# ingra14m/RobIR

Hardware: AMD Instinct MI355X
Metric: PBR-stage rays/sec (128 SG lobes, 32 visibility samples/lobe), full forward render (higher is better)
Workload: dtype f32 (every MLP -- light visibility, SDF values and reverse-mode gradient, colour, visibility, 512-wide and CESR nets: every fp32 operand exact as three f16 pieces, six MFMA products per multiply-add in three fp32 accumulators -- in the light-visibility kernel the two outer products of the 2^-22 clas

## Files before the change

robir_amd/csrc/vis_diffuse_x6t.hip:

```cpp
#include "../../include/robir_hip.h"
#include "common.h"
#include "mlp_engine.h"
#include "x6_ring.h"

namespace rb {

#define RB_TINY 1e-6f
constexpr int XT_MAX_DIRS = 4096;
constexpr int XT_WF4 = 1536;
constexpr int XT_CF4 = 4 + XT_WF4;
constexpr int XT_SLOTS = 4, XT_DIST = 3;
constexpr int XT_PIECES = 6;
#ifndef XT_FP8
#define XT_FP8 1
#endif

__device__ __forceinline__ void xt_dma16(const f4* gbase_uniform, unsigned lane_byte_off, unsigned lds_byte_uniform) {
  asm volatile("s_mov_b32 m0, %0\n\ts_nop 0\n\tglobal_load_lds_dwordx4 %1, %2" ::"s"(lds_byte_uniform), "v"(lane_byte_off),
               "s"(gbase_uniform)
               : "memory");
}
template <int OFF>
__device__ __forceinline__ void xt_dma16_imm(const f4* gbase_uniform, unsigned lane_byte_off, unsigned lds_byte_uniform) {
  asm volatile("s_mov_b32 m0, %0\n\ts_nop 0\n\tglobal_load_lds_dwordx4 %1, %2 offset:%3" ::"s"(lds_byte_uniform), "v"(lane_byte_off),
               "s"(gbase_uniform), "n"(OFF)
               : "memory");
}

template <int OFF>
__device__ __forceinline__ void xt_dma16_m0kept(const f4* gbase_uniform, unsigned lane_byte_off) {
  asm volatile("global_load_lds_dwordx4 %0, %1 offset:%2" ::"v"(lane_byte_off), "s"(gbase_uniform), "n"(OFF) : "memory");
}

struct XtTile {
  int point;
  int dir_base;
};
struct XtArgs {
  const float *A, *Bd;
  const f4* W49;
  int argmax_vis;
  unsigned* range_word;
  const float *normals, *dirs, *wdir, *wsum;
  const int* cid;
  int L, nsamp;
  float* vis_out;
  unsigned long long* eval_count;
  const unsigned short* pair_j;
  const XtTile* tile_info;
  const unsigned long long* counters;
  float* pair_vis;
};

template <bool STREAM>
__global__ __launch_bounds__(256, 1) void k_dvis_x6t(const XtArgs a) {
  __shared__ f4 ring[XT_SLOTS * XT_WF4];
  __shared__ f4 headw[XT_WF4];
  __shared__ f4 bias_tab[49 * 4];
  __shared__ f4 aux[(XT_MAX_DIRS * 4 + XT_MAX_DIRS * 2) / 16 + 64];
  __shared__ int s_count;
  float* const vis_tab = reinterpret_cast<float*>(aux);
  unsigned short* const idx_list = reinterpret_cast<unsigned short*>(aux + XT_MAX_DIRS / 4);
  f4* const a_row = aux + (XT_MAX_DIRS * 6) / 16;
  f4* const a_rows = aux;
  const float* __restrict__ A = a.A;
  const float* __restrict__ Bd = a.Bd;
  const f4* __restrict__ W49 = a.W49;
  const int argmax_vis = a.argmax_vis;
  const int tid = threadIdx.x, lane = tid & 63, g = lane >> 4;
  const int wave = __builtin_amdgcn_readfirstlane(tid >> 6);
  const float negk = -2048.0f;
  constexpr float C11 = 1.0f / 2048.0f;
  const long p = blockIdx.x;
  const int L = a.L, nsamp = a.nsamp, LS = L * nsamp;
  long dbase = 0;
  int S = 0, rounds = 0;
  const int G = gridDim.x;
  long total_tiles = 0, total_rounds = 0;
  for (int i = tid; i < 49 * 4; i += 256) bias_tab[i] = W49[(long)(i >> 2) * XT_CF4 + (i & 3)];
  for (int i = tid; i < XT_WF4; i += 256) headw[i] = W49[48L * XT_CF4 + 4 + i];
  if constexpr (STREAM) {
    total_tiles = (long)a.counters[0];
    total_rounds = (total_tiles + 7) >> 3;
    __syncthreads();
    if ((long)blockIdx.x >= total_rounds) return;
    rounds = 1;
  } else {
  const float* __restrict__ normals = a.normals;
  const float* __restrict__ dirs = a.dirs;
  const int* __restrict__ cid = a.cid;
  dbase = (cid ? (long)cid[p] : 0L) * LS;
  if (tid == 0) s_count = 0;
  if (tid < 64) a_row[tid] = reinterpret_cast<const f4*>(A + p * 256)[tid];
  for (int j = tid; j < LS; j += 256) vis_tab[j] = 0.f;
  __syncthreads();
  const float nx = normals[3 * p], ny = normals[3 * p + 1], nz = normals[3 * p + 2];
  for (int j0 = 0; j0 < LS; j0 += 256) {
    const int j = j0 + tid;
    bool front = false;
    if (j < LS) {
      const float* d = dirs + 3 * (dbase + j);
      const float c = nx * d[0] + ny * d[1] + nz * d[2];
      front = c > RB_TINY;
    }
    const unsigned long long mk = __ballot(front);
    int base = 0;
    if (lane == 0 && mk) base = atomicAdd(&s_count, __popcll(mk));
    base = __shfl(base, 0);
    if (front) idx_list[base + __popcll(mk & ((1ull << lane) - 1ull))] = (unsigned short)j;
  }
  __syncthreads();
  S = s_count;
  if (tid == 0 && a.eval_count) atomicAdd(a.eval_count, (unsigned long long)S);
  rounds = (S + 127) / 128;
  }

  const unsigned ring_b = (unsigned)(unsigned long)((__attribute__((address_space(3))) char*)ring);
  unsigned voff_a = (unsigned)wave * 6144u + (unsigned)lane * 16u, voff_b = voff_a + 4096u;
  asm volatile("" : "+v"(voff_a), "+v"(voff_b));
  const unsigned wave_lds = ring_b + (unsigned)wave * 6144u;
  typedef const __attribute__((address_space(3))) u4* lds_u4p;
  unsigned ring_a0 = ring_b + (unsigned)lane * 16u, ring_a2 = ring_a0 + 2u * XT_WF4 * 16u;
  asm volatile("" : "+v"(ring_a0), "+v"(ring_a2));
  const lds_u4p ring_u = (lds_u4p)ring_a0, ring_u2 = (lds_u4p)ring_a2;
  u4 wh[4], wm[4], wl[4];
#if XT_FP8
  typedef int xt_i8 __attribute__((ext_vector_type(8)));
  xt_i8 w8h, w8l;
#define XT_F16OFF(KB, PIECE) (((KB) >> 2) * 768 + (((KB) & 3) * 2 + (PIECE)) * 64)
#define XT_LOAD8(DST, BASE, OFF)                                                                                             \
  {                                                                                                                          \
    const u4 a_ = (BASE)[(OFF)], b_ = (BASE)[(OFF) + 64];                                                                    \
    DST = xt_i8{(int)a_[0], (int)a_[1], (int)a_[2], (int)a_[3], (int)b_[0], (int)b_[1], (int)b_[2], (int)b_[3]};             \
  }
#endif
  f4 bias;
  if (rounds > 0) {
#pragma unroll
    for (int c = 0; c < 3; ++c)
#pragma unroll
      for (int i = 0; i < XT_PIECES; ++i)
        xt_dma16(W49 + (long)c * XT_CF4 + 4 + i * 64, voff_a, wave_lds + (unsigned)c * 24576u + (unsigned)i * 1024u);
    asm volatile("s_waitcnt vmcnt(12)" ::: "memory");
    __builtin_amdgcn_s_barrier();
    asm volatile("" ::: "memory");
#pragma unroll
    for (int k = 0; k < 4; ++k) {
#if XT_FP8
      wh[k] = ring_u[XT_F16OFF(k, 0)];
      wm[k] = ring_u[XT_F16OFF(k, 1)];
#else
      wh[k] = ring_u[(k * 3 + 0) * 64];
      wm[k] = ring_u[(k * 3 + 1) * 64];
      wl[k] = ring_u[(k * 3 + 2) * 64];
#endif
    }
#if XT_FP8
    XT_LOAD8(w8h, ring_u, 512)
    XT_LOAD8(w8l, ring_u, 640)
#endif
    bias = bias_tab[g];
  }

  unsigned sat = 0u;
#if XT_FP8
  struct Ops {
    u4 h[2][8], m[2][8];
    xt_i8 h8[2][2], l8[2][2];
  };
  unsigned el_keep[2] = {0u, 0u};
#else
  struct Ops {
    u4 h[2][8], m[2][8], l[2][8];
  };
#endif
  Ops P, Q;

#define XT_MFMA(ACC, WREG, XREG) \
  ACC = __builtin_amdgcn_mfma_f32_16x16x32_f16(__builtin_bit_cast(h8, WREG), __builtin_bit_cast(h8, XREG), ACC, 0, 0, 0)

  float ev0[2][2], ev1[2][2], ed0, ed1;
  unsigned eh;
  SxAcc prev[2];
  auto ep_stage1 = [&](int t, int q) {
    const SxAcc& a = prev[t];
    const float r0 = __builtin_fmaf(__builtin_fmaf(a.c2[2 * q], C11, a.c1[2 * q]), C11, a.c0[2 * q]);
    const float r1 = __builtin_fmaf(__builtin_fmaf(a.c2[2 * q + 1], C11, a.c1[2 * q + 1]), C11, a.c0[2 * q + 1]);
    ev0[t][q] = fmaxf(r0, 0.f);
    ev1[t][q] = fmaxf(r1, 0.f);
  };
  auto ep_stage2 = [&](int t, int q) {
    const unsigned hu = __builtin_bit_cast(unsigned, __builtin_amdgcn_cvt_pkrtz(ev0[t][q], ev1[t][q]));
    const float s0 = ev0[t][q] * 2048.0f, s1 = ev1[t][q] * 2048.0f;
    asm("v_fma_mix_f32 %0, %1, %2, %3 op_sel_hi:[1,0,0]" : "=v"(ed0) : "v"(hu), "s"(negk), "v"(s0));
    asm("v_fma_mix_f32 %0, %1, %2, %3 op_sel:[1,0,0] op_sel_hi:[1,0,0]" : "=v"(ed1) : "v"(hu), "s"(negk), "v"(s1));
    eh = hu;
    sat = sat_acc_nonneg(sat, hu);
  };
  auto ep_stage3 = [&](Ops& Y, int t, int jb, int q) {
    const unsigned mu = __builtin_bit_cast(unsigned, __builtin_amdgcn_cvt_pkrtz(ed0, ed1));
    const float e0 = ed0 * 2048.0f, e1 = ed1 * 2048.0f;
    unsigned lu;
    asm("v_fma_mixlo_f16 %0, %1, %2, %3 op_sel_hi:[1,0,0]" : "=v"(lu) : "v"(mu), "s"(negk), "v"(e0));
    asm("v_fma_mixhi_f16 %0, %1, %2, %3 op_sel:[1,0,0] op_sel_hi:[1,0,0]" : "+v"(lu) : "v"(mu), "s"(negk), "v"(e1));
    Y.h[t][jb >> 1][(jb & 1) * 2 + q] = eh;
    Y.m[t][jb >> 1][(jb & 1) * 2 + q] = mu;
#if XT_FP8
    if (q == 0) {
      el_keep[t] = lu;
    } else {
      Y.h8[t][jb >> 3][jb & 7] = (int)__builtin_amdgcn_perm(eh, Y.h[t][jb >> 1][(jb & 1) * 2], 0x07050301u);
      Y.l8[t][jb >> 3][jb & 7] = (int)__builtin_amdgcn_perm(lu, el_keep[t], 0x07050301u);
    }
#else
    Y.l[t][jb >> 1][(jb & 1) * 2 + q] = lu;
#endif
  };
  auto ep_slot = [&](Ops& Y, int s, int pj) {
    switch (s) {
      case 0: ep_stage1(0, 0); break;
      case 1: ep_stage1(0, 1); break;
      case 2: ep_stage1(1, 0); break;
      case 3: ep_stage1(1, 1); break;
      case 4: ep_stage2(0, 0); break;
      case 5: ep_stage3(Y, 0, pj, 0); break;
      case 6: ep_stage2(0, 1); break;
      case 7: ep_stage3(Y, 0, pj, 1); break;
      case 8: ep_stage2(1, 0); break;
      case 9: ep_stage3(Y, 1, pj, 0); break;
      case 10: ep_stage2(1, 1); break;
      default: ep_stage3(Y, 1, pj, 1); break;
    }
  };

  f4 raw[2][16];
  int jj[2], jjn[2];
  int tpn[2] = {-1, -1}, tbn[2] = {0, 0}, jn2[2] = {0xFFFF, 0xFFFF};
  const unsigned arow_b = (unsigned)(unsigned long)((__attribute__((address_space(3))) char*)a_rows);
  XtTile recn[2] = {{-1, 0}, {-1, 0}};
  bool okn[2] = {false, false};
  auto tile_lookup = [&](long round) {
#pragma unroll
    for (int t = 0; t < 2; ++t) {
      const long T = round * 8 + wave * 2 + t;
      okn[t] = round < total_rounds && T < total_tiles;
      const long Tc = T < total_tiles ? T : total_tiles - 1;
      recn[t] = a.tile_info[Tc];
      jn2[t] = (int)a.pair_j[Tc * 16 + (lane & 15)];
    }
  };
  auto tile_resolve = [&]() {
#pragma unroll
    for (int t = 0; t < 2; ++t) {
      tpn[t] = okn[t] ? __builtin_amdgcn_readfirstlane(recn[t].point) : -1;
      tbn[t] = okn[t] ? __builtin_amdgcn_readfirstlane(recn[t].dir_base) : 0;
      if (!okn[t]) jn2[t] = 0xFFFF;
    }
  };
  auto fetch_rows = [&](long rd_next, int parity_next) {
    if constexpr (STREAM) {
      tile_resolve();
#pragma unroll
      for (int t = 0; t < 2; ++t) {
        const long prow = tpn[t] < 0 ? 0L : (long)tpn[t];
        xt_dma16(reinterpret_cast<const f4*>(A + prow * 256), (unsigned)lane * 16u,
                 arow_b + (unsigned)(parity_next * 8 + wave * 2 + t) * 1024u);
      }
    }
#pragma unroll
    for (int t = 0; t < 2; ++t) {
      long row;
      if constexpr (STREAM) {
        jjn[t] = (tpn[t] < 0 || jn2[t] == 0xFFFF) ? -1 : jn2[t];
        row = (long)tbn[t] + (jjn[t] < 0 ? 0 : jjn[t]);
      } else {
        const int si = (int)rd_next * 128 + t * 64 + wave * 16 + (lane & 15);
        jjn[t] = si < S ? (int)idx_list[si] : -1;
        row = dbase + (jjn[t] < 0 ? 0 : jjn[t]);
      }
      const f4* brow = reinterpret_cast<const f4*>(Bd + row * 256) + g;
#pragma unroll
      for (int kb = 0; kb < 16; ++kb) raw[t][kb] = brow[kb * 4];
    }
  };
  long rd = STREAM ? (long)blockIdx.x : 0L;
  const long rd_end = STREAM ? total_rounds : (long)rounds, rd_step = STREAM ? (long)G : 1L;
  int parity = 0;
  if constexpr (STREAM) tile_lookup(rd);
  if (rounds > 0) fetch_rows(rd, 0);
#ifdef XT_TIMING
#define XT_T(i) { const unsigned long long t_ = __builtin_amdgcn_s_memtime(); tacc[i] += t_ - tlast; tlast = t_; }
  unsigned long long tacc[4] = {0, 0, 0, 0}, tlast = __builtin_amdgcn_s_memtime();
  int trounds = 0;
#else
#define XT_T(i)
#endif
  for (; rd < rd_end; rd += rd_step) {
    if constexpr (STREAM) tile_lookup(rd + rd_step);
#ifdef XT_TIMING
    ++trounds;
#endif
    XT_T(3)
#pragma unroll
    for (int t = 0; t < 2; ++t) {
      jj[t] = jjn[t];
      const f4* arow = STREAM ? a_rows + (parity * 8 + wave * 2 + t) * 64 : a_row;
#pragma unroll
      for (int kb = 0; kb < 16; ++kb) {
        const f4 bv = raw[t][kb];
        const f4 av = arow[kb * 4 + g];
#pragma unroll
        for (int q = 0; q < 2; ++q) {
          unsigned h, m, l;
          sx_split_pair(fmaxf(av[2 * q] + bv[2 * q], 0.f), fmaxf(av[2 * q + 1] + bv[2 * q + 1], 0.f), negk, h, m, l);
          P.h[t][kb / 2][(kb & 1) * 2 + q] = h;
          P.m[t][kb / 2][(kb & 1) * 2 + q] = m;
#if XT_FP8
          if (q == 0) {
            el_keep[t] = l;
          } else {
            P.h8[t][kb >> 3][kb & 7] = (int)__builtin_amdgcn_perm(h, P.h[t][kb / 2][(kb & 1) * 2], 0x07050301u);
            P.l8[t][kb >> 3][kb & 7] = (int)__builtin_amdgcn_perm(l, el_keep[t], 0x07050301u);
          }
#else
          P.l[t][kb / 2][(kb & 1) * 2 + q] = l;
#endif
          sat = sat_acc_nonneg(sat, h);
        }
      }
    }
    XT_T(0)
    auto layer = [&](int l, Ops& X, Ops& Y) {
      const f4* Wl = W49 + (long)l * 16 * XT_CF4 + 4;
      const f4* Wn = W49 + (long)(l == 2 ? 0 : l + 1) * 16 * XT_CF4 + 4;
#pragma unroll
      for (int jb = 0; jb < 16; ++jb) {
        SxAcc acc[2];
        asm volatile("s_waitcnt vmcnt(6)" ::: "memory");
#ifndef XT_ABL_NOBAR
        __builtin_amdgcn_s_barrier();
#endif
        asm volatile("" ::: "memory");
        const int nx3 = jb + XT_DIST;
        const f4* dsrc = nx3 < 16 ? Wl + (long)nx3 * XT_CF4 : Wn + (long)(nx3 - 16) * XT_CF4;
        const unsigned ddst = wave_lds + (unsigned)(nx3 & 3) * 24576u;
        const f4 nbias = bias_tab[(l * 16 + jb + 1) * 4 + g];
#if defined(XT_ABL_NODMA)
#define XT_COPY(I) do { } while (0)
#else
#define XT_COPY(I)                                                                  \
  do {                                                                              \
    if ((I) == 0) xt_dma16_imm<0>(dsrc, voff_a, ddst);                              \
    else if ((I) < 4) xt_dma16_m0kept<((I) & 3) * 1024>(dsrc, voff_a);              \
    else if ((I) == 4) xt_dma16_imm<0>(dsrc, voff_b, ddst + 4096u);                 \
    else xt_dma16_m0kept<((I) & 3) * 1024>(dsrc, voff_b);                           \
  } while (0)
#endif
#define XT_FENCE __builtin_amdgcn_sched_barrier(0)
#ifdef XT_ABL_NOLDS
#define XT_FRAG(DST, KB, PIECE) asm volatile("" : "+v"(DST))
#else
#if XT_FP8
#define XT_FRAG(DST, KB, PIECE) DST = nfrag[XT_F16OFF(KB, PIECE)]
#else
#define XT_FRAG(DST, KB, PIECE) DST = nfrag[((KB) * 3 + (PIECE)) * 64]
#endif
#endif
#define XT_MFMA8(ACC, WREG, XREG) ACC = __builtin_amdgcn_mfma_scale_f32_16x16x128_f8f6f4(WREG, XREG, ACC, 1, 1, 0, 0, 0, 0)
#define XT_EP(S)                        \
  do {                                  \
    if (jb > 0) ep_slot(Y, (S), jb - 1); \
  } while (0)
#define XT_RUN(ACC, WP, XP)                     \
  _Pragma("unroll") for (int k_ = 0; k_ < 4; ++k_) { \
    const int k = H ? 3 - k_ : k_;               \
    XT_MFMA(ACC, WP[k], XP[4 * H + k]);          \
  }
#define XT_RUN_REFILL(ACC, WP, XP, PIECE)          \
  _Pragma("unroll") for (int k_ = 0; k_ < 4; ++k_) { \
    const int k = H ? 3 - k_ : k_;                   \
    XT_MFMA(ACC, WP[k], XP[4 * H + k]);              \
    XT_FRAG(WP[k], 4 * (1 - H) + k, PIECE);          \
  }
#pragma unroll
        for (int H = 0; H < 2; ++H) {
          const lds_u4p nfrag = (((jb + H) & 2) ? ring_u2 : ring_u) + ((jb + H) & 1) * XT_WF4;
          if (H == 0) {
            acc[0].c0 = bias;
            acc[1].c0 = bias;
            acc[0].c1 = acc[0].c2 = acc[1].c1 = acc[1].c2 = f4{0.f, 0.f, 0.f, 0.f};
          }
          XT_RUN(acc[0].c0, wh, X.h[0]);
          if (H == 0) XT_EP(0); else XT_EP(9);
          XT_FENCE;
          XT_RUN(acc[0].c1, wh, X.m[0]);
          if (H == 0) XT_EP(1); else XT_EP(10);
          XT_FENCE;
#if XT_FP8
          XT_MFMA8(acc[0].c2, w8h, X.l8[0][H]);
          if (H == 0) XT_EP(2); else XT_EP(11);
          XT_FENCE;
          XT_RUN(acc[1].c0, wh, X.h[1]);
          if (H == 0) XT_EP(3); else XT_COPY(0);
          XT_FENCE;
          XT_RUN_REFILL(acc[1].c1, wh, X.m[1], 0);
          XT_FENCE;
          XT_MFMA8(acc[1].c2, w8h, X.l8[1][H]);
#ifndef XT_ABL_NOLDS
          XT_LOAD8(w8h, nfrag, (1 - H) * 768 + 512)
#endif
          if (H == 0) XT_EP(4); else XT_COPY(1);
          XT_FENCE;
#else
          XT_RUN(acc[0].c2, wh, X.l[0]);
          if (H == 0) XT_EP(2); else XT_EP(11);
          XT_FENCE;
          XT_RUN(acc[1].c0, wh, X.h[1]);
          if (H == 0) XT_EP(3); else XT_COPY(0);
          XT_FENCE;
          XT_RUN(acc[1].c1, wh, X.m[1]);
          if (H == 0) XT_EP(4); else XT_COPY(1);
          XT_FENCE;
          XT_RUN_REFILL(acc[1].c2, wh, X.l[1], 0);
          XT_FENCE;
#endif
          XT_RUN(acc[0].c1, wm, X.h[0]);
          if (H == 0) XT_EP(5); else XT_COPY(2);
          XT_FENCE;
          XT_RUN(acc[0].c2, wm, X.m[0]);
          if (H == 0) XT_EP(6); else XT_COPY(3);
          XT_FENCE;
          XT_RUN(acc[1].c1, wm, X.h[1]);
          if (H == 0) XT_EP(7); else XT_COPY(4);
          XT_FENCE;
          XT_RUN_REFILL(acc[1].c2, wm, X.m[1], 1);
          XT_FENCE;
#if XT_FP8
          XT_MFMA8(acc[0].c2, w8l, X.h8[0][H]);
          if (H == 0) XT_EP(8); else XT_COPY(5);
          XT_FENCE;
          XT_MFMA8(acc[1].c2, w8l, X.h8[1][H]);
#ifndef XT_ABL_NOLDS
          XT_LOAD8(w8l, nfrag, (1 - H) * 768 + 640)
#endif
          XT_FENCE;
#else
          XT_RUN(acc[0].c2, wl, X.h[0]);
          if (H == 0) XT_EP(8); else XT_COPY(5);
          XT_FENCE;
          XT_RUN_REFILL(acc[1].c2, wl, X.h[1], 2);
          XT_FENCE;
#endif
        }
#undef XT_RUN
#undef XT_RUN_REFILL
#undef XT_COPY
#undef XT_FENCE
#undef XT_FRAG
#undef XT_MFMA8
#undef XT_EP
        prev[0] = acc[0];
        prev[1] = acc[1];
        bias = nbias;
      }
#pragma unroll
      for (int s = 0; s < 12; ++s) ep_slot(Y, s, 15);
    };
#pragma unroll 1
    for (int l = 0; l < 3; ++l) {
      layer(l, P, Q);
#pragma unroll
      for (int t = 0; t < 2; ++t)
#pragma unroll
        for (int kb = 0; kb < 8; ++kb) {
          P.h[t][kb] = Q.h[t][kb];
          P.m[t][kb] = Q.m[t][kb];
#if !XT_FP8
          P.l[t][kb] = Q.l[t][kb];
#endif
        }
#if XT_FP8
#pragma unroll
      for (int t = 0; t < 2; ++t)
#pragma unroll
        for (int hf = 0; hf < 2; ++hf) {
          P.h8[t][hf] = Q.h8[t][hf];
          P.l8[t][hf] = Q.l8[t][hf];
        }
#endif
    }
    XT_T(1)
    if constexpr (STREAM) fetch_rows(rd + rd_step, parity ^ 1);
    else fetch_rows(rd + 1 < rd_end ? rd + 1 : rd, 0);
    {
      const u4* hw = reinterpret_cast<const u4*>(headw) + lane;
      SxAcc acc[2];
#pragma unroll
      for (int t = 0; t < 2; ++t) {
        acc[t].c0 = bias;
        acc[t].c1 = f4{0.f, 0.f, 0.f, 0.f};
        acc[t].c2 = f4{0.f, 0.f, 0.f, 0.f};
      }
#pragma unroll
#if XT_FP8
      for (int kb = 0; kb < 8; ++kb) {
        const u4 fh = hw[XT_F16OFF(kb, 0)], fm = hw[XT_F16OFF(kb, 1)];
#pragma unroll
        for (int t = 0; t < 2; ++t) {
          XT_MFMA(acc[t].c0, fh, P.h[t][kb]);
          XT_MFMA(acc[t].c1, fh, P.m[t][kb]);
          XT_MFMA(acc[t].c1, fm, P.h[t][kb]);
          XT_MFMA(acc[t].c2, fm, P.m[t][kb]);
        }
      }
#pragma unroll
      for (int hf = 0; hf < 2; ++hf) {
        xt_i8 f8h, f8l;
        XT_LOAD8(f8h, hw, hf * 768 + 512)
        XT_LOAD8(f8l, hw, hf * 768 + 640)
#pragma unroll
        for (int t = 0; t < 2; ++t) {
          acc[t].c2 = __builtin_amdgcn_mfma_scale_f32_16x16x128_f8f6f4(f8h, P.l8[t][hf], acc[t].c2, 1, 1, 0, 0, 0, 0);
          acc[t].c2 = __builtin_amdgcn_mfma_scale_f32_16x16x128_f8f6f4(f8l, P.h8[t][hf], acc[t].c2, 1, 1, 0, 0, 0, 0);
        }
      }
#else
      for (int kb = 0; kb < 8; ++kb) {
        const u4 fh = hw[(kb * 3 + 0) * 64], fm = hw[(kb * 3 + 1) * 64], fl = hw[(kb * 3 + 2) * 64];
#pragma unroll
        for (int t = 0; t < 2; ++t) {
          XT_MFMA(acc[t].c0, fh, P.h[t][kb]);
          XT_MFMA(acc[t].c1, fh, P.m[t][kb]);
          XT_MFMA(acc[t].c2, fh, P.l[t][kb]);
          XT_MFMA(acc[t].c1, fm, P.h[t][kb]);
          XT_MFMA(acc[t].c2, fm, P.m[t][kb]);
          XT_MFMA(acc[t].c2, fl, P.h[t][kb]);
        }
      }
#endif
      bias = bias_tab[g];
#pragma unroll
      for (int t = 0; t < 2; ++t) {
        const float l0 = __builtin_fmaf(__builtin_fmaf(acc[t].c2[0], C11, acc[t].c1[0]), C11, acc[t].c0[0]);
        const float l1 = __builtin_fmaf(__builtin_fmaf(acc[t].c2[1], C11, acc[t].c1[1]), C11, acc[t].c0[1]);
        if (g == 0 && jj[t] >= 0) {
          float v;
          if (argmax_vis) {
            v = l1 > l0 ? 1.f : 0.f;
          } else {
            const float mx = fmaxf(l0, l1);
            const float e0 = expf(l0 - mx), e1 = expf(l1 - mx);
            v = e1 / (e0 + e1);
          }
          if constexpr (STREAM) a.pair_vis[(rd * 8 + wave * 2 + t) * 16 + (lane & 15)] = v;
          else vis_tab[jj[t]] = v;
        }
      }
    }
    parity ^= 1;
    XT_T(2)
  }
#ifdef XT_TIMING
  if ((blockIdx.x == 7 || blockIdx.x == 4000) && tid == 0 && trounds > 0)
    printf("x6t wg %d rounds %d cycles/round: conv %llu layers %llu head+fetch %llu lookup %llu\n", (int)blockIdx.x, trounds, tacc[0] / trounds,
           tacc[1] / trounds, tacc[2] / trounds, tacc[3] / trounds);
#endif
#undef XT_MFMA
  range_report<true>(sat, a.range_word);
  asm volatile("s_waitcnt vmcnt(0)" ::: "memory");
  __syncthreads();
  if constexpr (!STREAM) {
    if (tid < L) {
      const float* w = a.wdir + dbase + (long)tid * nsamp;
      float acc = 0.f;
      for (int k = 0; k < nsamp; ++k) acc += vis_tab[tid * nsamp + k] * w[k];
      a.vis_out[p * L + tid] = acc / a.wsum[(a.cid ? a.cid[p] : 0) * L + tid];
    }
  }
}

struct V3Tile;
__global__ void k_dvis3_cull(const float* __restrict__ normals, const int* __restrict__ cid, long n, const float* __restrict__ dirs, int LS,
                             unsigned short* __restrict__ pair_j, V3Tile* __restrict__ tile_info, int2* __restrict__ point_info,
                             unsigned long long* __restrict__ counters, unsigned long long* __restrict__ eval_count);
__global__ void k_dvis3_reduce(const int* __restrict__ cid, long n, const float* __restrict__ wdir, const float* __restrict__ wsum,
                               const unsigned short* __restrict__ pair_j, const float* __restrict__ pair_vis,
                               const int2* __restrict__ point_info, int L, int nsamp, float* __restrict__ vis_out);

}

using namespace rb;

extern "C" int rb_dvis_fused_x6t(const float* normals, const int* chunk_id, long n, const float* A, const float* Bd,
                                 const float* dirs, const float* wdir, const float* wsum, const float* W49, int L, int nsamp,
                                 int argmax_vis, int scale_log2, float* vis_out, unsigned long long* eval_count,
                                 rb_stream_t stream) {
  if (n <= 0) return 0;
  RB_REQUIRE(normals && A && Bd && dirs && wdir && wsum && W49 && vis_out, "null pointer");
  RB_REQUIRE(n <= RB_MAX_BLOCKS, "too many points for one launch (one workgroup each)");
  RB_REQUIRE(L > 0 && L <= 256 && nsamp > 0 && (long)L * nsamp <= XT_MAX_DIRS, "need L <= 256 and L*nsamp <= 4096");
#if XT_FP8
  RB_REQUIRE(scale_log2 == 8, "this build of k_dvis_x6t takes the bf8 weight layout (packing.repack_x6_chunks_fp8; scale_log2 = 8 names it)");
#else
  RB_REQUIRE(scale_log2 == 0, "k_dvis_x6t takes weights packed with scale_log2 = 0");
#endif
  XtArgs a{};
  a.A = A, a.Bd = Bd, a.W49 = (const f4*)W49, a.argmax_vis = argmax_vis;
  a.range_word = range_flags() ? range_flags() + RB_RANGE_DVIS : nullptr;
  a.normals = normals, a.dirs = dirs, a.wdir = wdir, a.wsum = wsum, a.cid = chunk_id, a.L = L, a.nsamp = nsamp;
  a.vis_out = vis_out, a.eval_count = eval_count;
  hipLaunchKernelGGL(k_dvis_x6t<false>, dim3((unsigned)n), dim3(256), 0, (hipStream_t)stream, a);
  return check_launch("k_dvis_x6t");
}

extern "C" int rb_dvis_stream_x6(const float* normals, const int* chunk_id, long n, const float* A, const float* Bd,
                                 const float* dirs, const float* wdir, const float* wsum, const float* W49, int L, int nsamp,
                                 int argmax_vis, int scale_log2, unsigned short* pair_j, float* pair_vis, int* tile_info,
                                 int* point_info, unsigned long long* counters, int n_workgroups, float* vis_out,
                                 unsigned long long* eval_count, rb_stream_t stream) {
  if (n <= 0) return 0;
  RB_REQUIRE(normals && A && Bd && dirs && wdir && wsum && W49 && vis_out, "null pointer");
  RB_REQUIRE(pair_j && pair_vis && tile_info && point_info && counters, "null scratch pointer");
  RB_REQUIRE(n <= RB_MAX_BLOCKS, "too many points for one launch (one workgroup each in the cull / reduce passes)");
  RB_REQUIRE(L > 0 && L <= 256 && nsamp > 0 && (long)L * nsamp <= XT_MAX_DIRS && (L * nsamp) % 16 == 0,
             "need L <= 256, L*nsamp <= 4096 and a multiple of 16");
  RB_REQUIRE((long)n * (L * nsamp / 16) < (1L << 31), "tile index would overflow 31 bits");
#if XT_FP8
  RB_REQUIRE(scale_log2 == 8, "this build of k_dvis_x6t takes the bf8 weight layout (packing.repack_x6_chunks_fp8; scale_log2 = 8 names it)");
#else
  RB_REQUIRE(scale_log2 == 0, "k_dvis_x6t takes weights packed with scale_log2 = 0");
#endif
  hipStream_t s = (hipStream_t)stream;
  if (n_workgroups <= 0) n_workgroups = device_cus();
  RB_REQUIRE(n_workgroups > 0, "device query failed");
  if (hipMemsetAsync(counters, 0, 2 * sizeof(unsigned long long), s) != hipSuccess) return rb::fail(__func__, "memset failed");
  hipLaunchKernelGGL(k_dvis3_cull, dim3((unsigned)n), dim3(256), 0, s, normals, chunk_id, n, dirs, L * nsamp, pair_j,
                     reinterpret_cast<V3Tile*>(tile_info), reinterpret_cast<int2*>(point_info), counters, eval_count);
  if (int rc = check_launch("k_dvis3_cull")) return rc;
  XtArgs a{};
  a.A = A, a.Bd = Bd, a.W49 = (const f4*)W49, a.argmax_vis = argmax_vis;
  a.range_word = range_flags() ? range_flags() + RB_RANGE_DVIS : nullptr;
  a.pair_j = pair_j, a.tile_info = reinterpret_cast<const XtTile*>(tile_info), a.counters = counters, a.pair_vis = pair_vis;
  hipLaunchKernelGGL(k_dvis_x6t<true>, dim3((unsigned)n_workgroups), dim3(256), 0, s, a);
  if (int rc = check_launch("k_dvis_x6t<stream>")) return rc;
  hipLaunchKernelGGL(k_dvis3_reduce, dim3((unsigned)n), dim3(256), 0, s, chunk_id, n, wdir, wsum, pair_j, pair_vis,
                     reinterpret_cast<const int2*>(point_info), L, nsamp, vis_out);
  return check_launch("k_dvis3_reduce");
}
```

Baseline: 510,000.

## Overlap weight DMA with culling prologue and parallelize the visibility reduction

In the non-stream path, the per-point prologue is restructured. Direction, head-weight, bias and A-row loads are issued together into registers, and the weight-ring DMA starts before culling so global latency overlaps. The LDS atomic compaction is replaced by per-wave ballot counts and a prefix over waves, which produces a deterministic ordered index list with fewer barriers. The epilogue multiplies by wdir across all 256 threads before a short per-lobe sum, replacing serial strided global reads. This adds register pressure from the prefetched arrays and only applies when LS is at most 4096.

```diff
diff --git a/robir_amd/csrc/vis_diffuse_x6t.hip b/robir_amd/csrc/vis_diffuse_x6t.hip
--- a/robir_amd/csrc/vis_diffuse_x6t.hip
+++ b/robir_amd/csrc/vis_diffuse_x6t.hip
@@ -7,6 +7,7 @@
 
 #define RB_TINY 1e-6f
 constexpr int XT_MAX_DIRS = 4096;
+constexpr int XT_CULL_IT = XT_MAX_DIRS / 256;
 constexpr int XT_WF4 = 1536;
 constexpr int XT_CF4 = 4 + XT_WF4;
 constexpr int XT_SLOTS = 4, XT_DIST = 3;
@@ -58,7 +59,7 @@
   __shared__ f4 headw[XT_WF4];
   __shared__ f4 bias_tab[49 * 4];
   __shared__ f4 aux[(XT_MAX_DIRS * 4 + XT_MAX_DIRS * 2) / 16 + 64];
-  __shared__ int s_count;
+  __shared__ int s_count[4];
   float* const vis_tab = reinterpret_cast<float*>(aux);
   unsigned short* const idx_list = reinterpret_cast<unsigned short*>(aux + XT_MAX_DIRS / 4);
   f4* const a_row = aux + (XT_MAX_DIRS * 6) / 16;
@@ -77,42 +78,76 @@
   int S = 0, rounds = 0;
   const int G = gridDim.x;
   long total_tiles = 0, total_rounds = 0;
-  for (int i = tid; i < 49 * 4; i += 256) bias_tab[i] = W49[(long)(i >> 2) * XT_CF4 + (i & 3)];
-  for (int i = tid; i < XT_WF4; i += 256) headw[i] = W49[48L * XT_CF4 + 4 + i];
+#ifdef XT_TIMING
+  const unsigned long long tstart = __builtin_amdgcn_s_memtime();
+#endif
+  auto ring_start = [&](unsigned voff, unsigned wlds) {
+#pragma unroll
+    for (int c = 0; c < 3; ++c)
+#pragma unroll
+      for (int i = 0; i < XT_PIECES; ++i)
+        xt_dma16(W49 + (long)c * XT_CF4 + 4 + i * 64, voff, wlds + (unsigned)c * 24576u + (unsigned)i * 1024u);
+  };
   if constexpr (STREAM) {
+    for (int i = tid; i < 49 * 4; i += 256) bias_tab[i] = W49[(long)(i >> 2) * XT_CF4 + (i & 3)];
+    for (int i = tid; i < XT_WF4; i += 256) headw[i] = W49[48L * XT_CF4 + 4 + i];
     total_tiles = (long)a.counters[0];
     total_rounds = (total_tiles + 7) >> 3;
     __syncthreads();
     if ((long)blockIdx.x >= total_rounds) return;
     rounds = 1;
   } else {
-  const float* __restrict__ normals = a.normals;
-  const float* __restrict__ dirs = a.dirs;
-  const int* __restrict__ cid = a.cid;
-  dbase = (cid ? (long)cid[p] : 0L) * LS;
-  if (tid == 0) s_count = 0;
-  if (tid < 64) a_row[tid] = reinterpret_cast<const f4*>(A + p * 256)[tid];
-  for (int j = tid; j < LS; j += 256) vis_tab[j] = 0.f;
-  __syncthreads();
-  const float nx = normals[3 * p], ny = normals[3 * p + 1], nz = normals[3 * p + 2];
-  for (int j0 = 0; j0 < LS; j0 += 256) {
-    const int j = j0 + tid;
-    bool front = false;
-    if (j < LS) {
-      const float* d = dirs + 3 * (dbase + j);
-      const float c = nx * d[0] + ny * d[1] + nz * d[2];
-      front = c > RB_TINY;
-    }
-    const unsigned long long mk = __ballot(front);
+    const float* __restrict__ normals = a.normals;
+    const float* __restrict__ dirs = a.dirs;
+    const int* __restrict__ cid = a.cid;
+    dbase = (cid ? (long)cid[p] : 0L) * LS;
+    ring_start((unsigned)wave * 6144u + (unsigned)lane * 16u,
+               (unsigned)(unsigned long)((__attribute__((address_space(3))) char*)ring) + (unsigned)wave * 6144u);
+    const float nx = normals[3 * p], ny = normals[3 * p + 1], nz = normals[3 * p + 2];
+    float dx[XT_CULL_IT], dy[XT_CULL_IT], dz[XT_CULL_IT];
+#pragma unroll
+    for (int it = 0; it < XT_CULL_IT; ++it) {
+      const int j = it * 256 + tid;
+      const float* d = dirs + 3 * (dbase + (j < LS ? j : LS - 1));
+      dx[it] = d[0], dy[it] = d[1], dz[it] = d[2];
+    }
+    f4 hw_r[XT_WF4 / 256];
+#pragma unroll
+    for (int k = 0; k < XT_WF4 / 256; ++k) hw_r[k] = W49[48L * XT_CF4 + 4 + k * 256 + tid];
+    const int bi = tid < 49 * 4 ? tid : 49 * 4 - 1;
+    const f4 bias_r = W49[(long)(bi >> 2) * XT_CF4 + (bi & 3)];
+    const f4 arow_r = reinterpret_cast<const f4*>(A + p * 256)[lane];
+    for (int j = tid; j < LS; j += 256) vis_tab[j] = 0.f;
+    unsigned long long mk[XT_CULL_IT];
+    int wave_count = 0;
+#pragma unroll
+    for (int it = 0; it < XT_CULL_IT; ++it) {
+      const float c = nx * dx[it] + ny * dy[it] + nz * dz[it];
+      mk[it] = __ballot(it * 256 + tid < LS && c > RB_TINY);
+      wave_count += __popcll(mk[it]);
+    }
+    if (lane == 0) s_count[wave] = wave_count;
+#pragma unroll
+    for (int k = 0; k < XT_WF4 / 256; ++k) headw[k * 256 + tid] = hw_r[k];
+    if (tid < 49 * 4) bias_tab[tid] = bias_r;
+    if (tid < 64) a_row[tid] = arow_r;
+    asm volatile("s_waitcnt vmcnt(0)" ::: "memory");
+    __syncthreads();
     int base = 0;
-    if (lane == 0 && mk) base = atomicAdd(&s_count, __popcll(mk));
-    base = __shfl(base, 0);
-    if (front) idx_list[base + __popcll(mk & ((1ull << lane) - 1ull))] = (unsigned short)j;
-  }
-  __syncthreads();
-  S = s_count;
-  if (tid == 0 && a.eval_count) atomicAdd(a.eval_count, (unsigned long long)S);
-  rounds = (S + 127) / 128;
+#pragma unroll
+    for (int w = 0; w < 4; ++w) {
+      const int c = s_count[w];
+      S += c;
+      base += w < wave ? c : 0;
+    }
+#pragma unroll
+    for (int it = 0; it < XT_CULL_IT; ++it) {
+      if ((mk[it] >> lane) & 1ull) idx_list[base + __popcll(mk[it] & ((1ull << lane) - 1ull))] = (unsigned short)(it * 256 + tid);
+      base += __popcll(mk[it]);
+    }
+    __syncthreads();
+    if (tid == 0 && a.eval_count) atomicAdd(a.eval_count, (unsigned long long)S);
+    rounds = (S + 127) / 128;
   }
 
   const unsigned ring_b = (unsigned)(unsigned long)((__attribute__((address_space(3))) char*)ring);
@@ -136,14 +171,12 @@
 #endif
   f4 bias;
   if (rounds > 0) {
-#pragma unroll
-    for (int c = 0; c < 3; ++c)
-#pragma unroll
-      for (int i = 0; i < XT_PIECES; ++i)
-        xt_dma16(W49 + (long)c * XT_CF4 + 4 + i * 64, voff_a, wave_lds + (unsigned)c * 24576u + (unsigned)i * 1024u);
-    asm volatile("s_waitcnt vmcnt(12)" ::: "memory");
-    __builtin_amdgcn_s_barrier();
-    asm volatile("" ::: "memory");
+    if constexpr (STREAM) {
+      ring_start(voff_a, wave_lds);
+      asm volatile("s_waitcnt vmcnt(12)" ::: "memory");
+      __builtin_amdgcn_s_barrier();
+      asm volatile("" ::: "memory");
+    }
 #pragma unroll
     for (int k = 0; k < 4; ++k) {
 #if XT_FP8
@@ -291,6 +324,7 @@
 #ifdef XT_TIMING
 #define XT_T(i) { const unsigned long long t_ = __builtin_amdgcn_s_memtime(); tacc[i] += t_ - tlast; tlast = t_; }
   unsigned long long tacc[4] = {0, 0, 0, 0}, tlast = __builtin_amdgcn_s_memtime();
+  const unsigned long long tprologue = tlast - tstart;
   int trounds = 0;
 #else
 #define XT_T(i)
@@ -561,22 +595,31 @@
     XT_T(2)
   }
 #ifdef XT_TIMING
-  if ((blockIdx.x == 7 || blockIdx.x == 4000) && tid == 0 && trounds > 0)
-    printf("x6t wg %d rounds %d cycles/round: conv %llu layers %llu head+fetch %llu lookup %llu\n", (int)blockIdx.x, trounds, tacc[0] / trounds,
-           tacc[1] / trounds, tacc[2] / trounds, tacc[3] / trounds);
+  const unsigned long long tloop_end = __builtin_amdgcn_s_memtime();
 #endif
 #undef XT_MFMA
   range_report<true>(sat, a.range_word);
   asm volatile("s_waitcnt vmcnt(0)" ::: "memory");
   __syncthreads();
   if constexpr (!STREAM) {
-    if (tid < L) {
-      const float* w = a.wdir + dbase + (long)tid * nsamp;
+    int tid_e = tid;
+    asm volatile("" : "+v"(tid_e));
+#pragma unroll 16
+    for (int j = tid_e; j < LS; j += 256) vis_tab[j] = vis_tab[j] * a.wdir[dbase + j];
+    __syncthreads();
+    if (tid_e < L) {
       float acc = 0.f;
-      for (int k = 0; k < nsamp; ++k) acc += vis_tab[tid * nsamp + k] * w[k];
-      a.vis_out[p * L + tid] = acc / a.wsum[(a.cid ? a.cid[p] : 0) * L + tid];
+      for (int k = 0; k < nsamp; ++k) acc += vis_tab[tid_e * nsamp + k];
+      a.vis_out[p * L + tid_e] = acc / a.wsum[(a.cid ? a.cid[p] : 0) * L + tid_e];
     }
   }
+#ifdef XT_TIMING
+  __syncthreads();
+  if ((blockIdx.x % 997 == 7) && tid == 0 && trounds > 0)
+    printf("x6t wg %d rounds %d S %d ticks: prologue %llu epilogue %llu | per round: lookup %llu conv %llu layers %llu head+fetch %llu\n",
+           (int)blockIdx.x, trounds, S, tprologue, __builtin_amdgcn_s_memtime() - tloop_end, tacc[3] / trounds, tacc[0] / trounds,
+           tacc[1] / trounds, tacc[2] / trounds);
+#endif
 }
 
 struct V3Tile;
```

Result: no change. 511,200, median of 6 (+0.3%).
